# RobotLocomotion/pytorch-dense-correspondence

Measured on NVIDIA H100. Metric: image-pairs/s (640x480, D=3) fwd+loss+bwd, higher is better.
Workload: dtype f32 (bf16x3 split on the wgmma tensor cores, fp32 accumulate)

## Files before the change

pytorch-dense-correspondence_b200/csrc/conv_tc.cu:

```cuda
#include <cuda.h>
#include <algorithm>
#include <cstdlib>
#include <cstring>
#include <functional>
#include <mutex>
#include <unordered_map>

#include "conv.cuh"
#include "conv_tc.cuh"

namespace ddn {

constexpr int TC_BLOCK_K = 64;
constexpr int TC_CONSUMERS = 256;
constexpr int TC_THREADS = TC_CONSUMERS + 32;
constexpr int TC_PRODUCER_WARP = TC_CONSUMERS / 32;
constexpr int TC_WIDE_THREADS = TC_CONSUMERS + 128;
constexpr int TC_A_BYTES = 128 * TC_BLOCK_K * 2;

__device__ __forceinline__ uint32_t smem_u32(const void* p) { return (uint32_t)__cvta_generic_to_shared(p); }

__device__ __forceinline__ void mbar_init(uint32_t bar, uint32_t count) {
  asm volatile("mbarrier.init.shared::cta.b64 [%0], %1;" ::"r"(bar), "r"(count));
}
// ... 115 lines not shown
  } else {
    Wgmma<N>::template mma<TRANS>(d, a_hi, b_hi, accumulate);
  }
}
template <int N, int TRANS, int NPROD>
__device__ __forceinline__ void mma_k16_x(float (&d)[N / 2], float (&x)[N / 2], uint64_t a_hi, uint64_t a_lo, uint64_t b_hi, uint64_t b_lo,
                                          int accumulate) {
  if (NPROD == 3) {
    Wgmma<N>::template mma<TRANS>(x, a_hi, b_lo, accumulate);
    Wgmma<N>::template mma<TRANS>(x, a_lo, b_hi, 1);
  }
  Wgmma<N>::template mma<TRANS>(d, a_hi, b_hi, accumulate);
}
template <int K>
__device__ __forceinline__ void add_cross(float (&d)[K], const float (&x)[K]) {
#pragma unroll
  for (int i = 0; i < K; ++i) d[i] += x[i];
}
template <int N, int K>
__device__ __forceinline__ float (&acc_cols(float (&d)[K]))[N / 2] {
  static_assert(N / 2 <= K, "accumulator too narrow");
  return *reinterpret_cast<float(*)[N / 2]>(&d[0]);
}

constexpr int EPI_ROWS = 4;
constexpr int EPI_STRIDE = 40;
constexpr int EPI_WARP_FLOATS = 16 * EPI_STRIDE;

template <int K>
__device__ __forceinline__ void stage_write(const float (&acc)[K], int c, float* st, int lane) {
  const int r = lane >> 2, q = (lane & 3) * 2;
#pragma unroll
  for (int jj = 0; jj < 4; ++jj) {
    const int j = 4 * c + jj;
    *reinterpret_cast<float2*>(st + r * EPI_STRIDE + 8 * jj + q) = make_float2(acc[4 * j], acc[4 * j + 1]);
    *reinterpret_cast<float2*>(st + (r + 8) * EPI_STRIDE + 8 * jj + q) = make_float2(acc[4 * j + 2], acc[4 * j + 3]);
  }
  __syncwarp();
}

template <int K>
__device__ __forceinline__ void stage_chunk(const float (&acc)[K], int c, float* st, int lane, float4 (&v)[EPI_ROWS]) {
  stage_write(acc, c, st, lane);
  const int ga = lane >> 3, gb = lane & 7;
#pragma unroll
  for (int i = 0; i < EPI_ROWS; ++i) v[i] = *reinterpret_cast<const float4*>(st + (EPI_ROWS * ga + i) * EPI_STRIDE + 4 * gb);
  __syncwarp();
}

__device__ __forceinline__ uint32_t pack_bf16x2(__nv_bfloat16 a, __nv_bfloat16 b) {
  return (uint32_t)__bfloat16_as_ushort(a) | ((uint32_t)__bfloat16_as_ushort(b) << 16);
}

template <typename P>
__device__ __forceinline__ void conv_epilogue_rows(const P& p, const float4 (&v)[EPI_ROWS], size_t off, size_t rs, int n_ok, int ch,
                                                   int C, int grp, float4& s1, float4& s2) {
  float4 adv[EPI_ROWS];
#pragma unroll
  for (int i = 0; i < EPI_ROWS; ++i)
    adv[i] = (p.addend && i < n_ok) ? __ldg(reinterpret_cast<const float4*>(p.addend + off + i * rs)) : make_float4(0.f, 0.f, 0.f, 0.f);
  if (p.ep_scale) {
    const float4 sc = __ldg(reinterpret_cast<const float4*>(p.ep_scale + ch));
    const float4 sh = __ldg(reinterpret_cast<const float4*>(p.ep_shift + ch));
#pragma unroll
    for (int i = 0; i < EPI_ROWS; ++i) {
      float4 f = make_float4(fmaf(v[i].x, sc.x, sh.x) + adv[i].x, fmaf(v[i].y, sc.y, sh.y) + adv[i].y,
                             fmaf(v[i].z, sc.z, sh.z) + adv[i].z, fmaf(v[i].w, sc.w, sh.w) + adv[i].w);
      if (p.ep_relu) { f.x = fmaxf(f.x, 0.f); f.y = fmaxf(f.y, 0.f); f.z = fmaxf(f.z, 0.f); f.w = fmaxf(f.w, 0.f); }
      if (i < n_ok) {
        if (p.out) *reinterpret_cast<float4*>(p.out + off + i * rs) = f;
        if (p.out_hi) {
          const __nv_bfloat16 h0 = __float2bfloat16_rn(f.x), h1 = __float2bfloat16_rn(f.y), h2 = __float2bfloat16_rn(f.z), h3 = __float2bfloat16_rn(f.w);
          *reinterpret_cast<uint2*>(p.out_hi + off + i * rs) = make_uint2(pack_bf16x2(h0, h1), pack_bf16x2(h2, h3));
          if (p.out_lo)
            *reinterpret_cast<uint2*>(p.out_lo + off + i * rs) =
                make_uint2(pack_bf16x2(__float2bfloat16_rn(f.x - __bfloat162float(h0)), __float2bfloat16_rn(f.y - __bfloat162float(h1))),
                           pack_bf16x2(__float2bfloat16_rn(f.z - __bfloat162float(h2)), __float2bfloat16_rn(f.w - __bfloat162float(h3))));
        }
      }
    }
  } else if (p.bst.fin.a.acc) {
    float4 rw[EPI_ROWS];
    uint2 yh[EPI_ROWS];
#pragma unroll
    for (int i = 0; i < EPI_ROWS; ++i) {
      rw[i] = i < n_ok ? __ldg(reinterpret_cast<const float4*>(p.bst.raw + off + i * rs)) : make_float4(0.f, 0.f, 0.f, 0.f);
      if (p.bst.y_hi) yh[i] = i < n_ok ? __ldg(reinterpret_cast<const uint2*>(p.bst.y_hi + off + i * rs)) : make_uint2(0u, 0u);
    }
    const float4 mu = __ldg(reinterpret_cast<const float4*>(p.bst.mean + (size_t)grp * C + ch));
    const float4 is = __ldg(reinterpret_cast<const float4*>(p.bst.invstd + (size_t)grp * C + ch));
    float4 scl = make_float4(0.f, 0.f, 0.f, 0.f), be = scl;
    if (!p.bst.y_hi && p.bst.relu) {
      const float4 gm = __ldg(reinterpret_cast<const float4*>(p.bst.gamma + ch));
      be = __ldg(reinterpret_cast<const float4*>(p.bst.beta + ch));
      scl = make_float4(gm.x * is.x, gm.y * is.y, gm.z * is.z, gm.w * is.w);
    }
#pragma unroll
    for (int i = 0; i < EPI_ROWS; ++i) {
      float4 g = make_float4(v[i].x + adv[i].x, v[i].y + adv[i].y, v[i].z + adv[i].z, v[i].w + adv[i].w);
      if (i < n_ok) *reinterpret_cast<float4*>(p.out + off + i * rs) = g;
      else g = make_float4(0.f, 0.f, 0.f, 0.f);
      if (p.bst.y_hi) {
        const uint2 hh = yh[i];
        if ((hh.x & 0x8000u) || !(hh.x & 0x7fffu)) g.x = 0.f;
        if ((hh.x & 0x80000000u) || !(hh.x & 0x7fff0000u)) g.y = 0.f;
        if ((hh.y & 0x8000u) || !(hh.y & 0x7fffu)) g.z = 0.f;
        if ((hh.y & 0x80000000u) || !(hh.y & 0x7fff0000u)) g.w = 0.f;
      } else if (p.bst.relu) {
        if (!(fmaf(rw[i].x - mu.x, scl.x, be.x) > 0.f)) g.x = 0.f;
        if (!(fmaf(rw[i].y - mu.y, scl.y, be.y) > 0.f)) g.y = 0.f;
        if (!(fmaf(rw[i].z - mu.z, scl.z, be.z) > 0.f)) g.z = 0.f;
        if (!(fmaf(rw[i].w - mu.w, scl.w, be.w) > 0.f)) g.w = 0.f;
      }
      s1.x += g.x; s1.y += g.y; s1.z += g.z; s1.w += g.w;
      s2.x = fmaf(g.x, (rw[i].x - mu.x) * is.x, s2.x); s2.y = fmaf(g.y, (rw[i].y - mu.y) * is.y, s2.y);
      s2.z = fmaf(g.z, (rw[i].z - mu.z) * is.z, s2.z); s2.w = fmaf(g.w, (rw[i].w - mu.w) * is.w, s2.w);
    }
  } else {
#pragma unroll
    for (int i = 0; i < EPI_ROWS; ++i) {
      const float4 raw = i < n_ok ? v[i] : make_float4(0.f, 0.f, 0.f, 0.f);
      if (i < n_ok)
        *reinterpret_cast<float4*>(p.out + off + i * rs) = make_float4(raw.x + adv[i].x, raw.y + adv[i].y, raw.z + adv[i].z, raw.w + adv[i].w);
      s1.x += raw.x; s1.y += raw.y; s1.z += raw.z; s1.w += raw.w;
      s2.x = fmaf(raw.x, raw.x, s2.x); s2.y = fmaf(raw.y, raw.y, s2.y); s2.z = fmaf(raw.z, raw.z, s2.z); s2.w = fmaf(raw.w, raw.w, s2.w);
    }
  }
}

__device__ __forceinline__ void colsum_lane_groups(float4& s1, float4& s2) {
#pragma unroll
  for (int off = 8; off < 32; off <<= 1) {
    s1.x += __shfl_xor_sync(0xffffffffu, s1.x, off); s1.y += __shfl_xor_sync(0xffffffffu, s1.y, off);
    s1.z += __shfl_xor_sync(0xffffffffu, s1.z, off); s1.w += __shfl_xor_sync(0xffffffffu, s1.w, off);
    s2.x += __shfl_xor_sync(0xffffffffu, s2.x, off); s2.y += __shfl_xor_sync(0xffffffffu, s2.y, off);
    s2.z += __shfl_xor_sync(0xffffffffu, s2.z, off); s2.w += __shfl_xor_sync(0xffffffffu, s2.w, off);
  }
}

__device__ __forceinline__ void named_barrier(int id, int threads) { asm volatile("bar.sync %0, %1;" ::"r"(id), "r"(threads) : "memory"); }

struct TcConvParams {
  float* out;
  const float* addend;
  int N, H, W, Cin, Cout;
  int taps_w;
  int dil;
  int stride;
  int tiles_h, tiles_w;
  int n_sub;
  int n_co;
  int full_items, tail_split, total_items;
  int imgs_per_group;
  BnFwdFinal fin;
  TcBwdStats bst;
  const float* ep_scale; const float* ep_shift; int ep_relu;
  __nv_bfloat16* out_hi; __nv_bfloat16* out_lo;
};

constexpr int TC_SUB_H = 4, TC_SUB_W = 16;
constexpr int TC_SUB_BYTES = 64 * 128;

struct TcItem { int sp, co0, width; };
__device__ __forceinline__ TcItem tc_item(const TcConvParams& p, int idx, int block_n) {
  int tile = idx, piece = 0, width = block_n;
  if (idx >= p.full_items) {
    const int j = idx - p.full_items;
    tile = p.full_items + j / p.tail_split;
    piece = j - (j / p.tail_split) * p.tail_split;
    width = block_n / p.tail_split;
  }
  TcItem it;
  it.sp = tile / p.n_co;
  it.co0 = (tile - it.sp * p.n_co) * block_n + piece * width;
  it.width = width;
  return it;
}
struct TcSub { int n, h0, w0; bool valid; };
__device__ __forceinline__ TcSub tc_sub(const TcConvParams& p, int st) {
  TcSub s;
  s.valid = st < p.n_sub;
  const int tw = st % p.tiles_w; const int t = st / p.tiles_w;
  const int th = t % p.tiles_h;
  s.n = s.valid ? t / p.tiles_h : p.N;
  s.h0 = th * TC_SUB_H; s.w0 = tw * TC_SUB_W;
  return s;
}

template <int W, int BLOCK_N, int NPROD, int STAGES, int TRANS = 0>
__device__ __forceinline__ void conv_tc_mainloop(float (&acc)[W / 2], float (&accx)[W / 2], int num_kb, uint32_t& g, const uint64_t* full_bar,
                                                 const uint64_t* empty_bar, const uint8_t* smem, int wg, int lane) {
  constexpr int NSPLIT = NPROD == 3 ? 2 : 1;
  constexpr int A_BYTES = 128 * TC_BLOCK_K * 2;
  constexpr int B_BYTES = BLOCK_N * TC_BLOCK_K * 2;
  constexpr int STAGE_BYTES = NSPLIT * (A_BYTES + B_BYTES);
  constexpr uint32_t LBO = TRANS ? TC_SUB_BYTES : 16;
  constexpr int K_STEP = TRANS ? 16 * 128 : 32;
  for (int kb = 0; kb < num_kb; ++kb, ++g) {
    const int s = g % STAGES;
    mbar_wait(smem_u32(&full_bar[s]), (g / STAGES) & 1);
    wgmma_fence();
    const uint32_t stg = smem_u32(smem + (size_t)s * STAGE_BYTES);
    const uint64_t a_hi = gmma_desc(stg + wg * TC_SUB_BYTES, LBO, 1024), a_lo = gmma_desc(stg + A_BYTES + wg * TC_SUB_BYTES, LBO, 1024);
    const uint64_t b_hi = gmma_desc(stg + NSPLIT * A_BYTES, LBO, 1024), b_lo = gmma_desc(stg + 2 * A_BYTES + B_BYTES, LBO, 1024);
#pragma unroll
    for (int k = 0; k < TC_BLOCK_K / 16; ++k) {
      const uint64_t adv = (uint64_t)((k * K_STEP) >> 4);
      mma_k16_x<W, TRANS, NPROD>(acc, accx, a_hi + adv, a_lo + adv, b_hi + adv, b_lo + adv, (kb | k) != 0);
    }
    wgmma_commit();
    wgmma_wait<1>();
    if (kb > 0 && lane == 0) mbar_arrive(smem_u32(&empty_bar[(g - 1) % STAGES]));
  }
  wgmma_wait<0>();
  fence_acc(acc);
  if (NPROD == 3) { fence_acc(accx); add_cross(acc, accx); }
  if (lane == 0) mbar_arrive(smem_u32(&empty_bar[(g - 1) % STAGES]));
}

template <int BLOCK_N, int NPROD>
__global__ void __launch_bounds__(TC_WIDE_THREADS, 1)
conv_tc_kernel(const __grid_constant__ CUtensorMap tm_a_hi, const __grid_constant__ CUtensorMap tm_a_lo,
               const __grid_constant__ CUtensorMap tm_b_hi, const __grid_constant__ CUtensorMap tm_b_lo,
               const __grid_constant__ CUtensorMap tm_bt_hi, const __grid_constant__ CUtensorMap tm_bt_lo,
               const TcConvParams p) {
  constexpr int NSPLIT = NPROD == 3 ? 2 : 1;
  constexpr int A_BYTES = 128 * TC_BLOCK_K * 2;
  constexpr int B_BYTES = BLOCK_N * TC_BLOCK_K * 2;
  constexpr int STAGE_BYTES = NSPLIT * (A_BYTES + B_BYTES);
  constexpr int STAGES = (192 * 1024) / STAGE_BYTES >= 8 ? 8 : (192 * 1024) / STAGE_BYTES;
  static_assert(STAGES >= 2, "pipeline needs at least two stages");

  extern __shared__ __align__(1024) uint8_t smem_raw[];
  uint8_t* smem = reinterpret_cast<uint8_t*>((reinterpret_cast<uintptr_t>(smem_raw) + 1023) & ~uintptr_t(1023));
  __shared__ __align__(8) uint64_t full_bar[STAGES];
  __shared__ __align__(8) uint64_t empty_bar[STAGES];
  __shared__ int s_last;
  __shared__ __align__(16) float s_stage[TC_CONSUMERS / 32][EPI_WARP_FLOATS];
  __shared__ __align__(16) float s_part[2][2][4][BLOCK_N];

  pdl_trigger();
  const int warp = __shfl_sync(0xffffffffu, threadIdx.x >> 5, 0), lane = threadIdx.x & 31;
  const int cin_chunks = p.Cin / TC_BLOCK_K;
  const int num_kb = p.taps_w * p.taps_w * cin_chunks;
  const int half = p.taps_w >> 1;

  if (threadIdx.x == 0) {
    for (int s = 0; s < STAGES; ++s) { mbar_init(smem_u32(&full_bar[s]), 1); mbar_init(smem_u32(&empty_bar[s]), TC_CONSUMERS / 32); }
    fence_barrier_init();
    tma_prefetch_desc(&tm_a_hi); tma_prefetch_desc(&tm_b_hi); tma_prefetch_desc(&tm_bt_hi);
    if (NSPLIT == 2) { tma_prefetch_desc(&tm_a_lo); tma_prefetch_desc(&tm_b_lo); tma_prefetch_desc(&tm_bt_lo); }
  }
  __syncthreads();
  pdl_wait();

  if (warp >= TC_PRODUCER_WARP) {
    setmaxnreg_dec<40>();
    if (warp == TC_PRODUCER_WARP && lane == 0) {
      uint32_t g = 0;
      for (int idx = blockIdx.x; idx < p.total_items; idx += gridDim.x) {
        const TcItem it = tc_item(p, idx, BLOCK_N);
        const bool tail = it.width != BLOCK_N;
        const uint32_t stage_tx = (uint32_t)(NSPLIT * (A_BYTES + it.width * TC_BLOCK_K * 2));
        const CUtensorMap* mb_hi = tail ? &tm_bt_hi : &tm_b_hi;
        const CUtensorMap* mb_lo = tail ? &tm_bt_lo : &tm_b_lo;
        const TcSub s0 = tc_sub(p, it.sp * 2), s1 = tc_sub(p, it.sp * 2 + 1);
        for (int kb = 0; kb < num_kb; ++kb, ++g) {
          const int s = g % STAGES;
          mbar_wait(smem_u32(&empty_bar[s]), ((g / STAGES) & 1) ^ 1);
          const int tap = kb / cin_chunks, cc = kb - tap * cin_chunks;
          const int r = tap / p.taps_w, sx = tap - r * p.taps_w;
          const int dh = (r - half) * p.dil, dw = (sx - half) * p.dil;
          uint8_t* stg = smem + (size_t)s * STAGE_BYTES;
          const uint32_t bar = smem_u32(&full_bar[s]);
          mbar_expect_tx(bar, stage_tx);
          tma_load_4d(smem_u32(stg), &tm_a_hi, bar, cc * TC_BLOCK_K, s0.w0 * p.stride + dw, s0.h0 * p.stride + dh, s0.n);
          tma_load_4d(smem_u32(stg + TC_SUB_BYTES), &tm_a_hi, bar, cc * TC_BLOCK_K, s1.w0 * p.stride + dw, s1.h0 * p.stride + dh, s1.n);
          tma_load_2d(smem_u32(stg + NSPLIT * A_BYTES), mb_hi, bar, kb * TC_BLOCK_K, it.co0);
          if (NSPLIT == 2) {
            tma_load_4d(smem_u32(stg + A_BYTES), &tm_a_lo, bar, cc * TC_BLOCK_K, s0.w0 * p.stride + dw, s0.h0 * p.stride + dh, s0.n);
            tma_load_4d(smem_u32(stg + A_BYTES + TC_SUB_BYTES), &tm_a_lo, bar, cc * TC_BLOCK_K, s1.w0 * p.stride + dw, s1.h0 * p.stride + dh, s1.n);
            tma_load_2d(smem_u32(stg + 2 * A_BYTES + B_BYTES), mb_lo, bar, kb * TC_BLOCK_K, it.co0);
          }
        }
      }
    }
  } else {
    setmaxnreg_inc<232>();
    const int wg = warp >> 2, w = warp & 3, e = threadIdx.x & 127;
    const int ga = lane >> 3, gb = lane & 7;
    const bool stats = p.fin.a.acc != nullptr;
    const bool bstats = p.bst.fin.a.acc != nullptr;
    double* const sum_acc = bstats ? p.bst.fin.a.acc : p.fin.a.acc;
    float* const st = s_stage[warp];
    float acc[BLOCK_N / 2], accx[BLOCK_N / 2];
    uint32_t g = 0;
    for (int idx = blockIdx.x; idx < p.total_items; idx += gridDim.x) {
      const TcItem it = tc_item(p, idx, BLOCK_N);
      if (it.width == BLOCK_N)
        conv_tc_mainloop<BLOCK_N, BLOCK_N, NPROD, STAGES>(acc, accx, num_kb, g, full_bar, empty_bar, smem, wg, lane);
      else if (BLOCK_N > 64 && it.width == 64)
        conv_tc_mainloop<64, BLOCK_N, NPROD, STAGES>(acc_cols<64>(acc), acc_cols<64>(accx), num_kb, g, full_bar, empty_bar, smem, wg, lane);
      else
        conv_tc_mainloop<32, BLOCK_N, NPROD, STAGES>(acc_cols<32>(acc), acc_cols<32>(accx), num_kb, g, full_bar, empty_bar, smem, wg, lane);

      const TcSub sb = tc_sub(p, it.sp * 2 + wg);
      const int h = sb.h0 + w, w4 = sb.w0 + EPI_ROWS * ga;
      const int n_ok = (sb.valid && h < p.H) ? min(EPI_ROWS, p.W - w4) : 0;
      const size_t pix = ((size_t)(n_ok > 0 ? sb.n : 0) * p.H + (n_ok > 0 ? h : 0)) * p.W + (n_ok > 0 ? w4 : 0);
      const size_t cbase = pix * p.Cout + it.co0 + gb * 4;
      const int grp = sb.valid ? sb.n / p.imgs_per_group : 0;
#pragma unroll
      for (int c = 0; c < BLOCK_N / 32; ++c) {
        if (c < (it.width >> 5)) {
          float4 v[EPI_ROWS];
          stage_chunk(acc, c, st, lane, v);
          float4 s1 = make_float4(0.f, 0.f, 0.f, 0.f), s2 = s1;
          conv_epilogue_rows(p, v, cbase + c * 32, (size_t)p.Cout, n_ok, it.co0 + c * 32 + gb * 4, p.Cout, grp, s1, s2);
          if (stats || bstats) {
            colsum_lane_groups(s1, s2);
            if (ga == 0) {
              *reinterpret_cast<float4*>(&s_part[wg][0][w][c * 32 + gb * 4]) = s1;
              *reinterpret_cast<float4*>(&s_part[wg][1][w][c * 32 + gb * 4]) = s2;
            }
          }
        }
      }
      if (stats || bstats) {
        named_barrier(1 + wg, 128);
        if (sb.valid)
          for (int col = e; col < it.width; col += 128) {
#pragma unroll
            for (int k = 0; k < 2; ++k) {
              const float sum = s_part[wg][k][0][col] + s_part[wg][k][1][col] + s_part[wg][k][2][col] + s_part[wg][k][3][col];
              red_add_f64(sum_acc + (size_t)(grp * 2 + k) * p.Cout + it.co0 + col, (double)sum);
            }
          }
        named_barrier(1 + wg, 128);
      }
    }
    if (stats) {
      const bool last = bn_last_cta(p.fin.a.ticket, gridDim.x, threadIdx.x == 0, &s_last, [] { named_barrier(3, TC_CONSUMERS); });
      if (last)
        for (int c = threadIdx.x; c < p.Cout; c += TC_CONSUMERS) bn_fwd_finalize_channel(p.fin, c);
    } else if (bstats) {
      const bool last = bn_last_cta(p.bst.fin.a.ticket, gridDim.x, threadIdx.x == 0, &s_last, [] { named_barrier(3, TC_CONSUMERS); });
      if (last)
        for (int c = threadIdx.x; c < p.Cout; c += TC_CONSUMERS) bn_bwd_finalize_channel(p.bst.fin, c);
    }
  }
}

struct TcHaloParams {
  float* out; const float* addend;
  int N, H, W;
  int tiles_h, tiles_w, n_tiles;
  int imgs_per_group;
  BnFwdFinal fin;
  TcBwdStats bst;
  const float* ep_scale; const float* ep_shift; int ep_relu;
  __nv_bfloat16* out_hi; __nv_bfloat16* out_lo;
};
constexpr int HALO_TH = 8, HALO_TW = 16;
constexpr int HALO_BH = HALO_TH + 2, HALO_BW = HALO_TW + 2;
constexpr int HALO_BOX_BYTES = HALO_BH * HALO_BW * 128;
constexpr int HALO_SLOT = ((HALO_BOX_BYTES + 1023) / 1024) * 1024;
constexpr int HALO_B_TAP = 64 * 128;
constexpr int HALO_B_PLANE = 9 * HALO_B_TAP;
__host__ __device__ constexpr int halo_slots(int nprod) { return nprod == 3 ? 2 : 3; }

template <int NPROD>
__global__ void __launch_bounds__(TC_THREADS, 1)
conv64_halo_kernel(const __grid_constant__ CUtensorMap tm_a_hi, const __grid_constant__ CUtensorMap tm_a_lo,
                   const __grid_constant__ CUtensorMap tm_b_hi, const __grid_constant__ CUtensorMap tm_b_lo, const TcHaloParams p) {
  constexpr int NSPLIT = NPROD == 3 ? 2 : 1;
  constexpr int SLOTS = halo_slots(NPROD);
  extern __shared__ __align__(1024) uint8_t smem_raw[];
  uint8_t* smem = reinterpret_cast<uint8_t*>((reinterpret_cast<uintptr_t>(smem_raw) + 1023) & ~uintptr_t(1023));
  uint8_t* smem_b = smem;
  uint8_t* smem_a = smem + NSPLIT * HALO_B_PLANE;
  __shared__ __align__(8) uint64_t full_bar[SLOTS], empty_bar[SLOTS], b_full;
  __shared__ int s_last;
  __shared__ __align__(16) float s_stage[TC_CONSUMERS / 32][EPI_WARP_FLOATS];
  __shared__ __align__(16) float s_part[2][8][64];

  pdl_trigger();
  const int warp = __shfl_sync(0xffffffffu, threadIdx.x >> 5, 0), lane = threadIdx.x & 31;
  if (threadIdx.x == 0) {
    for (int s = 0; s < SLOTS; ++s) { mbar_init(smem_u32(&full_bar[s]), 1); mbar_init(smem_u32(&empty_bar[s]), TC_CONSUMERS / 32); }
    mbar_init(smem_u32(&b_full), 1);
    fence_barrier_init();
    tma_prefetch_desc(&tm_a_hi); tma_prefetch_desc(&tm_b_hi);
    if (NSPLIT == 2) { tma_prefetch_desc(&tm_a_lo); tma_prefetch_desc(&tm_b_lo); }
  }
  __syncthreads();
  pdl_wait();

  auto tile_of = [&](int t, int& n, int& h0, int& w0) {
    const int tw = t % p.tiles_w; const int q = t / p.tiles_w;
    const int th = q % p.tiles_h; n = q / p.tiles_h;
    h0 = th * HALO_TH; w0 = tw * HALO_TW;
  };

  if (warp == TC_PRODUCER_WARP) {
    if (lane == 0) {
      const uint32_t bb = smem_u32(&b_full);
      mbar_expect_tx(bb, NSPLIT * HALO_B_PLANE);
#pragma unroll 1
      for (int tap = 0; tap < 9; ++tap) {
        tma_load_2d(smem_u32(smem_b + tap * HALO_B_TAP), &tm_b_hi, bb, tap * 64, 0);
        if (NSPLIT == 2) tma_load_2d(smem_u32(smem_b + HALO_B_PLANE + tap * HALO_B_TAP), &tm_b_lo, bb, tap * 64, 0);
      }
      uint32_t g = 0;
      constexpr int PF = 2;
      for (int j = 0; j < PF; ++j) {
        const int tp = blockIdx.x + j * gridDim.x;
        if (tp < p.n_tiles) {
          int n, h0, w0;
          tile_of(tp, n, h0, w0);
          tma_prefetch_l2_4d(&tm_a_hi, 0, h0 - 1, w0 - 1, n);
          if (NSPLIT == 2) tma_prefetch_l2_4d(&tm_a_lo, 0, h0 - 1, w0 - 1, n);
        }
      }
      for (int t = blockIdx.x; t < p.n_tiles; t += gridDim.x) {
        int n, h0, w0;
        {
          const int tp = t + PF * gridDim.x;
          if (tp < p.n_tiles) {
            tile_of(tp, n, h0, w0);
            tma_prefetch_l2_4d(&tm_a_hi, 0, h0 - 1, w0 - 1, n);
            if (NSPLIT == 2) tma_prefetch_l2_4d(&tm_a_lo, 0, h0 - 1, w0 - 1, n);
          }
        }
        tile_of(t, n, h0, w0);
#pragma unroll
        for (int pl = 0; pl < NSPLIT; ++pl, ++g) {
          const int s = g % SLOTS;
          mbar_wait(smem_u32(&empty_bar[s]), ((g / SLOTS) & 1) ^ 1);
          const uint32_t bar = smem_u32(&full_bar[s]);
          mbar_expect_tx(bar, HALO_BOX_BYTES);
          tma_load_4d(smem_u32(smem_a + s * HALO_SLOT), pl == 0 ? &tm_a_hi : &tm_a_lo, bar, 0, h0 - 1, w0 - 1, n);
        }
      }
    }
  } else {
    const int wg = warp >> 2, w = warp & 3;
    const int ga = lane >> 3, gb = lane & 7;
    const bool stats = p.fin.a.acc != nullptr;
    const bool bstats = p.bst.fin.a.acc != nullptr;
    double* const sum_acc = bstats ? p.bst.fin.a.acc : p.fin.a.acc;
    float* const st = s_stage[warp];
    mbar_wait(smem_u32(&b_full), 0);
    const uint64_t bd_hi = gmma_desc_k(smem_u32(smem_b));
    const uint64_t bd_lo = gmma_desc_k(smem_u32(smem_b + HALO_B_PLANE));
    const uint32_t a_wg = (uint32_t)(8 * wg * HALO_BH * 128);
    float acc[32], accx[32];
    uint32_t g = 0;
    for (int t = blockIdx.x; t < p.n_tiles; t += gridDim.x) {
      int n, h0, w0;
      tile_of(t, n, h0, w0);
      const int s_hi = g % SLOTS;
      {
        mbar_wait(smem_u32(&full_bar[s_hi]), (g / SLOTS) & 1);
        wgmma_fence();
        const uint64_t a0 = gmma_desc_k(smem_u32(smem_a + s_hi * HALO_SLOT) + a_wg, HALO_BH * 128);
#pragma unroll
        for (int tap = 0; tap < 9; ++tap) {
#pragma unroll
          for (int k = 0; k < 4; ++k) {
            const uint64_t ad = a0 + (uint64_t)((((tap % 3) * HALO_BH + tap / 3) * 128 + k * 32) >> 4);
            const uint64_t boff = (uint64_t)((tap * HALO_B_TAP + k * 32) >> 4);
            if (NPROD == 3) Wgmma<64>::mma<0>(accx, ad, bd_lo + boff, (tap | k) != 0);
            Wgmma<64>::mma<0>(acc, ad, bd_hi + boff, (tap | k) != 0);
          }
        }
        wgmma_commit();
        ++g;
      }
      if (NPROD == 3) {
        const int s = g % SLOTS;
        mbar_wait(smem_u32(&full_bar[s]), (g / SLOTS) & 1);
        const uint64_t a0 = gmma_desc_k(smem_u32(smem_a + s * HALO_SLOT) + a_wg, HALO_BH * 128);
#pragma unroll
        for (int tap = 0; tap < 9; ++tap) {
#pragma unroll
          for (int k = 0; k < 4; ++k)
            Wgmma<64>::mma<0>(accx, a0 + (uint64_t)((((tap % 3) * HALO_BH + tap / 3) * 128 + k * 32) >> 4),
                              bd_hi + (uint64_t)((tap * HALO_B_TAP + k * 32) >> 4), 1);
        }
        wgmma_commit();
        wgmma_wait<1>();
        if (lane == 0) mbar_arrive(smem_u32(&empty_bar[s_hi]));
        ++g;
      }
      wgmma_wait<0>();
      fence_acc(acc);
      if (NPROD == 3) { fence_acc(accx); add_cross(acc, accx); }
      if (lane == 0) mbar_arrive(smem_u32(&empty_bar[(g - 1) % SLOTS]));

      const size_t pix0 = ((size_t)n * p.H + h0 + EPI_ROWS * (ga & 1)) * p.W + (w0 + 8 * wg + 2 * w + (ga >> 1));
      const size_t row_stride = (size_t)p.W * 64;
      const int grp = n / p.imgs_per_group;
#pragma unroll
      for (int c = 0; c < 2; ++c) {
        float4 v[EPI_ROWS];
        stage_chunk(acc, c, st, lane, v);
        float4 s1 = make_float4(0.f, 0.f, 0.f, 0.f), s2 = s1;
        conv_epilogue_rows(p, v, pix0 * 64 + gb * 4 + c * 32, row_stride, EPI_ROWS, c * 32 + gb * 4, 64, grp, s1, s2);
        if (stats || bstats) {
          colsum_lane_groups(s1, s2);
          if (ga == 0) {
            *reinterpret_cast<float4*>(&s_part[0][warp][c * 32 + gb * 4]) = s1;
            *reinterpret_cast<float4*>(&s_part[1][warp][c * 32 + gb * 4]) = s2;
          }
        }
      }
      if (stats || bstats) {
        named_barrier(3, TC_CONSUMERS);
        if (threadIdx.x < 128) {
          const int col = threadIdx.x & 63, k = threadIdx.x >> 6;
          float s8 = 0.f;
#pragma unroll
          for (int q = 0; q < 8; ++q) s8 += s_part[k][q][col];
          red_add_f64(sum_acc + (size_t)(grp * 2 + k) * 64 + col, (double)s8);
        }
        named_barrier(3, TC_CONSUMERS);
      }
    }
    if (bstats) {
      const bool last = bn_last_cta(p.bst.fin.a.ticket, gridDim.x, threadIdx.x == 0, &s_last, [] { named_barrier(3, TC_CONSUMERS); });
      if (last)
        for (int c = threadIdx.x; c < 64; c += TC_CONSUMERS) bn_bwd_finalize_channel(p.bst.fin, c);
    } else if (stats) {
      const bool last = bn_last_cta(p.fin.a.ticket, gridDim.x, threadIdx.x == 0, &s_last, [] { named_barrier(3, TC_CONSUMERS); });
      if (last)
        for (int c = threadIdx.x; c < 64; c += TC_CONSUMERS) bn_fwd_finalize_channel(p.fin, c);
    }
  }
}

struct TcWgradParams {
  double* dwp;
  int N, H, W, Cin, Cout;
  int taps_w, dil, stride;
  int tiles_h, tiles_w;
  int total_kb;
  int n_co, n_ci, n_tiles;
  int chunks;
};

struct WgradItem { int co0, ci0, tap, kb0, kb1; };
__device__ __forceinline__ WgradItem wgrad_item(const TcWgradParams& p, int idx, int bn) {
  const int c = idx / p.n_tiles;
  int t = idx - c * p.n_tiles;
  WgradItem it;
  it.co0 = (t % p.n_co) * 128; t /= p.n_co;
  it.ci0 = (t % p.n_ci) * bn;
  it.tap = t / p.n_ci;
  it.kb0 = (int)((int64_t)c * p.total_kb / p.chunks);
  it.kb1 = (int)((int64_t)(c + 1) * p.total_kb / p.chunks);
  return it;
// ... 641 lines not shown
  return fold != 0;
}

bool tc_conv_supported(int Cin, int Cout, int k, int stride, int pad, int dil, int H, int W) {
  if (Cin % 64 || Cout % 64) return false;
  if (stride == 2) { if (dil != 1 || (H & 1) || (W & 1)) return false; }
  else if (stride != 1) return false;
  if (k == 3) return pad == dil;
  if (k == 1) return pad == 0;
  return false;
}

static const size_t kMaxWeightElems = (size_t)9 * 512 * 512;
size_t tc_weight_ws_bytes() { return 2 * align_up(kMaxWeightElems * 2, 1024) + 2048; }

int tc_split(const float* x, __nv_bfloat16* hi, __nv_bfloat16* lo, int64_t n, int precision, cudaStream_t st) {
  DDN_CHECK_ARG(n % 4 == 0, "split: element count must be a multiple of 4");
  int64_t n4 = n / 4;
  int blocks = (int)std::min<int64_t>(ceil_div(n4, 256), (int64_t)num_sms() * 8);
  DDN_LAUNCH(split_bf16_kernel, blocks, 256, 0, st, x, hi, lo, n4, precision == DDN_PRECISION_BF16X3 ? 1 : 0);
  return 0;
}

int tc_pack_weights(const float* w_oihw, __nv_bfloat16* hi, __nv_bfloat16* lo, int Cout, int Cin, int k, int dgrad, int precision,
                    cudaStream_t st) {
  const size_t wel = (size_t)Cout * Cin * k * k;
  int wblocks = (int)std::min<int64_t>(ceil_div((int64_t)wel, 256), 4096);
  DDN_LAUNCH(pack_weights_tc_kernel, wblocks, 256, 0, st, w_oihw, hi, lo, Cout, Cin, k, dgrad, precision == DDN_PRECISION_BF16X3 ? 1 : 0);
  return 0;
}

int tc_upsample_zero_split(const float* dy, __nv_bfloat16* hi, __nv_bfloat16* lo, int N, int Ho, int Wo, int C, int precision,
                           cudaStream_t st) {
  int64_t total = (int64_t)N * Ho * Wo * (C / 4);
  int blocks = (int)std::min<int64_t>(ceil_div(total, 256), (int64_t)num_sms() * 8);
  DDN_LAUNCH(upsample_zero_split_kernel, blocks, 256, 0, st, dy, hi, lo, N, Ho, Wo, C, precision == DDN_PRECISION_BF16X3 ? 1 : 0);
  return 0;
}

int tc_stem_patches(const float* x_nchw, __nv_bfloat16* hi, __nv_bfloat16* lo, int N, int H, int W, int precision, cudaStream_t st) {
  const int H1 = (H - 1) / 2 + 1, W1 = (W - 1) / 2 + 1;
  DDN_CHECK_ARG(N <= 65535 && H1 <= 65535, "stem: batch / height too large for the launch grid");
  dim3 grid((unsigned)ceil_div(W1, STEM_TW), (unsigned)H1, (unsigned)N);
  DDN_LAUNCH(stem_patch_split_kernel, grid, 256, 0, st, x_nchw, hi, lo, N, H, W, H1, W1, precision == DDN_PRECISION_BF16X3 ? 1 : 0);
  return 0;
}

static bool tc_tail_enabled() {
  static int v = -1;
  if (v < 0) { const char* e = getenv("DDN_TC_TAIL"); v = (e && e[0] == '0') ? 0 : 1; }
  return v != 0;
}

template <int BLOCK_N, int NPROD>
static int launch_conv_tc(const CUtensorMap& a_hi, const CUtensorMap& a_lo, const CUtensorMap& b_hi, const CUtensorMap& b_lo,
                          const CUtensorMap& bt_hi, const CUtensorMap& bt_lo, const TcConvParams& p, int workers, cudaStream_t st) {
  constexpr int NSPLIT = NPROD == 3 ? 2 : 1;
  constexpr int STAGE_BYTES = NSPLIT * (128 * TC_BLOCK_K * 2 + BLOCK_N * TC_BLOCK_K * 2);
  constexpr int STAGES = (192 * 1024) / STAGE_BYTES >= 8 ? 8 : (192 * 1024) / STAGE_BYTES;
  const size_t smem = (size_t)STAGES * STAGE_BYTES + 1024;
  static bool configured = false;
  if (!configured) {
    DDN_CUDA(cudaFuncSetAttribute(conv_tc_kernel<BLOCK_N, NPROD>, cudaFuncAttributeMaxDynamicSharedMemorySize, (int)smem));
    configured = true;
  }
  DDN_LAUNCH((conv_tc_kernel<BLOCK_N, NPROD>), workers, TC_WIDE_THREADS, smem, st, a_hi, a_lo, b_hi, b_lo, bt_hi, bt_lo, p);
  return 0;
}

template <int NPROD>
static int launch_conv64_halo(const CUtensorMap& a_hi, const CUtensorMap& a_lo, const CUtensorMap& b_hi, const CUtensorMap& b_lo,
                              const TcHaloParams& p, cudaStream_t st) {
  constexpr int NSPLIT = NPROD == 3 ? 2 : 1;
  const size_t smem = (size_t)NSPLIT * HALO_B_PLANE + (size_t)halo_slots(NPROD) * HALO_SLOT + 1024;
  static bool configured = false;
  if (!configured) {
    DDN_CUDA(cudaFuncSetAttribute(conv64_halo_kernel<NPROD>, cudaFuncAttributeMaxDynamicSharedMemorySize, (int)smem));
    configured = true;
  }
  const int grid = std::min(p.n_tiles, tc_worker_sms());
  DDN_LAUNCH((conv64_halo_kernel<NPROD>), grid, TC_THREADS, smem, st, a_hi, a_lo, b_hi, b_lo, p);
  return 0;
}

int tc_conv_planes(TcPlanes in, const float* w_oihw, const TcPlanes* wpk, float* out, const float* addend, const BnFwdFinal* stats,
                   int N, int H, int W, int Cin, int Cout, int k, int stride, int dil, int dgrad, int precision,
                   void* wws, size_t wws_bytes, cudaStream_t st, const TcFoldedEpilogue* ep, const TcBwdStats* bst) {
  DDN_CHECK_ARG(stride == 1 || !dgrad, "the strided data gradient goes through zero-inserted planes (stride 1 here)");
  const int Ho = H / stride, Wo = W / stride;
  const double fl = 2.0 * N * Ho * Wo * (double)Cout * k * k * Cin;
  const int gin = dgrad ? Cout : Cin, gout = dgrad ? Cin : Cout;
  const int want_lo = precision == DDN_PRECISION_BF16X3;
  const __nv_bfloat16* b_hi; const __nv_bfloat16* b_lo;
  if (wpk) {
    b_hi = wpk->hi; b_lo = wpk->lo;
  } else {
    const size_t wel = (size_t)Cout * Cin * k * k;
    const size_t w_b = align_up(kMaxWeightElems * 2, 1024);
    DDN_CHECK_ARG(wws != nullptr && wel <= kMaxWeightElems, "tc weight staging missing or weight tensor too large");
    char* base = reinterpret_cast<char*>(align_up(reinterpret_cast<uintptr_t>(wws), 1024));
    if ((size_t)(base - (char*)wws) + 2 * w_b > wws_bytes) { set_error("tensor-core weight staging too small"); return DDN_EWORKSPACE; }
    __nv_bfloat16* ph = (__nv_bfloat16*)base; __nv_bfloat16* pl = (__nv_bfloat16*)(base + w_b);
    int wblocks = (int)std::min<int64_t>(ceil_div((int64_t)wel, 256), 4096);
    DDN_LAUNCH(pack_weights_tc_kernel, wblocks, 256, 0, st, w_oihw, ph, pl, Cout, Cin, k, dgrad, want_lo);
    b_hi = ph; b_lo = pl;
  }
  if (tc_halo_enabled() && k == 3 && gin == 64 && gout == 64 && stride == 1 && dil == 1 && Ho % HALO_TH == 0 && Wo % HALO_TW == 0) {
    TcHaloParams hp;
    memset(&hp, 0, sizeof(hp));
    if (ep) {
      DDN_CHECK_ARG(!dgrad && !stats && !bst && ep->scale && ep->shift && (out || ep->out_hi), "folded epilogue: forward only, needs scale/shift and an output");
      hp.ep_scale = ep->scale; hp.ep_shift = ep->shift; hp.ep_relu = ep->relu; hp.out_hi = ep->out_hi; hp.out_lo = want_lo ? ep->out_lo : nullptr;
    } else {
      DDN_CHECK_ARG(out != nullptr, "conv output pointer is null");
    }
    hp.out = out; hp.addend = addend; hp.N = N; hp.H = Ho; hp.W = Wo;
    hp.tiles_h = Ho / HALO_TH; hp.tiles_w = Wo / HALO_TW; hp.n_tiles = N * hp.tiles_h * hp.tiles_w;
    hp.imgs_per_group = N;
    if (stats) {
      DDN_CHECK_ARG(!dgrad && stats->G >= 1 && stats->G <= BN_MAX_GROUPS && N % stats->G == 0 && stats->C == 64, "bad BatchNorm statistics request");
      hp.fin = *stats;
      hp.imgs_per_group = N / stats->G;
    }
    if (bst) {
      DDN_CHECK_ARG(dgrad && !stats && bst->raw && bst->mean && bst->invstd && bst->fin.a.acc && bst->fin.G >= 1 && bst->fin.G <= BN_MAX_GROUPS &&
                    N % bst->fin.G == 0 && bst->fin.C == 64 && (bst->y_hi || !bst->relu || (bst->gamma && bst->beta)),
                    "bad BatchNorm backward-statistics request");
      hp.bst = *bst;
      hp.imgs_per_group = N / bst->fin.G;
    }
    CUtensorMap ma_hi, ma_lo, mb_hi, mb_lo;
    DDN_TRY(make_act_map_halo(&ma_hi, in.hi, N, H, W, 64));
    DDN_TRY(make_act_map_halo(&ma_lo, want_lo ? in.lo : in.hi, N, H, W, 64));
    DDN_TRY(make_weight_map(&mb_hi, b_hi, 64, 9 * 64, 64));
    DDN_TRY(make_weight_map(&mb_lo, want_lo ? b_lo : b_hi, 64, 9 * 64, 64));
    ProfScope ps(dgrad ? PROF_CONV_DGRAD_TC : PROF_CONV_FWD_TC, fl, st);
    return want_lo ? launch_conv64_halo<3>(ma_hi, ma_lo, mb_hi, mb_lo, hp, st) : launch_conv64_halo<1>(ma_hi, ma_lo, mb_hi, mb_lo, hp, st);
  }
  const int block_n = gout % 128 == 0 ? 128 : 64;
  TcConvParams p;
  memset(&p, 0, sizeof(p));
  p.out = out; p.addend = addend; p.N = N; p.H = Ho; p.W = Wo; p.Cin = gin; p.Cout = gout; p.taps_w = k; p.dil = dil;
  p.stride = stride;
  p.tiles_h = (int)ceil_div(Ho, TC_SUB_H); p.tiles_w = (int)ceil_div(Wo, TC_SUB_W);
  p.n_sub = N * p.tiles_h * p.tiles_w;
  p.n_co = gout / block_n;
  const int tiles = (int)ceil_div(p.n_sub, 2) * p.n_co;
  const int workers_max = tc_worker_sms();
  const int rem = tiles % workers_max;
  int split = 1;
  if (rem && tc_tail_enabled())
    while (split * 2 <= 8 && block_n / (split * 2) >= 32 && rem * split * 2 <= workers_max) split *= 2;
  p.full_items = tiles - rem; p.tail_split = split; p.total_items = p.full_items + rem * split;
  if (split == 1) { p.full_items = tiles; p.total_items = tiles; }
  const int workers = std::min(p.total_items, workers_max);
  p.imgs_per_group = N;
  if (stats) {
    DDN_CHECK_ARG(!dgrad && !ep && stats->G >= 1 && stats->G <= BN_MAX_GROUPS && N % stats->G == 0, "bad BatchNorm statistics request");
    p.fin = *stats;
    p.imgs_per_group = N / stats->G;
  }
  if (bst) {
    DDN_CHECK_ARG(dgrad && !ep && !stats && bst->raw && bst->mean && bst->invstd && bst->fin.a.acc && bst->fin.G >= 1 &&
                  bst->fin.G <= BN_MAX_GROUPS && N % bst->fin.G == 0 && bst->fin.C == gout && (bst->y_hi || !bst->relu || (bst->gamma && bst->beta)),
                  "bad BatchNorm backward-statistics request");
    p.bst = *bst;
    p.imgs_per_group = N / bst->fin.G;
  }
  if (ep) {
    DDN_CHECK_ARG(!dgrad && !stats && ep->scale && ep->shift && (out || ep->out_hi), "folded epilogue: forward only, needs scale/shift and an output");
    p.ep_scale = ep->scale; p.ep_shift = ep->shift; p.ep_relu = ep->relu; p.out_hi = ep->out_hi; p.out_lo = want_lo ? ep->out_lo : nullptr;
  } else {
    DDN_CHECK_ARG(out != nullptr, "conv output pointer is null");
  }
  const int b_rows = block_n;
  const int bt_rows = b_rows / split;
  CUtensorMap ma_hi, ma_lo, mb_hi, mb_lo, mt_hi, mt_lo;
  DDN_TRY(make_act_map(&ma_hi, in.hi, N, H, W, gin, stride));
  DDN_TRY(make_act_map(&ma_lo, want_lo ? in.lo : in.hi, N, H, W, gin, stride));
  DDN_TRY(make_weight_map(&mb_hi, b_hi, gout, k * k * gin, b_rows));
  DDN_TRY(make_weight_map(&mb_lo, want_lo ? b_lo : b_hi, gout, k * k * gin, b_rows));
  DDN_TRY(make_weight_map(&mt_hi, b_hi, gout, k * k * gin, bt_rows));
  DDN_TRY(make_weight_map(&mt_lo, want_lo ? b_lo : b_hi, gout, k * k * gin, bt_rows));
  ProfScope ps(dgrad ? PROF_CONV_DGRAD_TC : PROF_CONV_FWD_TC, fl, st);
#define CONV_TC(BN)                                                                                                           \
  (want_lo ? launch_conv_tc<BN, 3>(ma_hi, ma_lo, mb_hi, mb_lo, mt_hi, mt_lo, p, workers, st)                                   \
           : launch_conv_tc<BN, 1>(ma_hi, ma_lo, mb_hi, mb_lo, mt_hi, mt_lo, p, workers, st))
  if (block_n == 128) return CONV_TC(128);
  return CONV_TC(64);
#undef CONV_TC
}

int tc_dgrad_strided(const float* dy_f32, TcPlanes up, const float* w_oihw, const TcPlanes* w_packed, float* dx, const float* addend,
                     int N, int H, int W, int Cin, int Cout, int k, int precision, void* wws, size_t wws_bytes, cudaStream_t st,
                     const TcBwdStats* bst) {
  DDN_TRY(tc_upsample_zero_split(dy_f32, const_cast<__nv_bfloat16*>(up.hi), const_cast<__nv_bfloat16*>(up.lo), N, H / 2, W / 2, Cout,
                                 precision, st));
  return tc_conv_planes(up, w_oihw, w_packed, dx, addend, nullptr, N, H, W, Cin, Cout, k, 1, 1, 1, precision, wws, wws_bytes, st, nullptr, bst);
}

int tc_stem_pack_weights(const float* w_conv1, __nv_bfloat16* hi, __nv_bfloat16* lo, int precision, cudaStream_t st) {
  DDN_LAUNCH(stem_pack_weights_kernel, (64 * 192 + 255) / 256, 256, 0, st, w_conv1, hi, lo, precision == DDN_PRECISION_BF16X3 ? 1 : 0);
  return 0;
}
int tc_stem_forward(TcPlanes patches, const float* w_conv1, const TcPlanes* w_packed, float* raw, const BnFwdFinal* stats, int N, int H1,
                    int W1, int precision, void* wws, size_t wws_bytes, cudaStream_t st) {
  TcPlanes wpk;
  if (w_packed) wpk = *w_packed;
  else {
    char* base = reinterpret_cast<char*>(align_up(reinterpret_cast<uintptr_t>(wws), 1024));
    DDN_CHECK_ARG((size_t)(base - (char*)wws) + 2 * 64 * 192 * 2 + 1024 <= wws_bytes, "weight staging too small");
    __nv_bfloat16* ph = (__nv_bfloat16*)base; __nv_bfloat16* pl = (__nv_bfloat16*)(base + align_up((size_t)64 * 192 * 2, 1024));
    DDN_TRY(tc_stem_pack_weights(w_conv1, ph, pl, precision, st));
    wpk.hi = ph; wpk.lo = pl;
  }
  return tc_conv_planes(patches, nullptr, &wpk, raw, nullptr, stats, N, H1, W1, 192, 64, 1, 1, 1, 0, precision, wws, wws_bytes, st);
}

int tc_stem_wgrad(TcPlanes patches, TcPlanes dy, float* dw_conv1, int N, int H1, int W1, int precision, double* scratch, cudaStream_t st) {
  if (!dw_conv1) return tc_wgrad_planes(patches, dy, nullptr, N, H1, W1, 192, 64, 1, 1, 1, precision, scratch, st);
  double* dwp = scratch; float* dwk = reinterpret_cast<float*>(scratch + 64 * 192);
  DDN_TRY(tc_wgrad_planes(patches, dy, dwk, N, H1, W1, 192, 64, 1, 1, 1, precision, dwp, st));
  DDN_LAUNCH(stem_unpack_wgrad_kernel, (64 * 147 + 255) / 256, 256, 0, st, dwk, dw_conv1);
  return 0;
}

int tc_pack_all(const float* params, int64_t n_params, char* cache, const TcPackEntry* entries, int n, unsigned long long* fp_new,
                unsigned long long* fp_old, int force, int precision, cudaStream_t st) {
  DDN_CHECK_ARG(n >= 1 && n <= TC_PACK_MAX, "pack table too large");
  TcPackTable t; t.n = n;
  for (int i = 0; i < n; ++i) t.e[i] = entries[i];
  DDN_LAUNCH(param_fingerprint_kernel, num_sms() * 2, 256, 0, st, reinterpret_cast<const uint32_t*>(params), n_params, fp_new);
  dim3 grid(32, (unsigned)n);
  DDN_LAUNCH(pack_all_kernel, grid, 256, 0, st, params, cache, t, fp_new, fp_old, force, precision == DDN_PRECISION_BF16X3 ? 1 : 0);
  DDN_LAUNCH(commit_fingerprint_kernel, 1, 32, 0, st, fp_new, fp_old);
  return 0;
}

size_t tc_workspace_bytes(size_t max_act_elems) { return tc_weight_ws_bytes() + 6 * align_up(max_act_elems * 2, 1024) + 4096; }

// ... 45 lines not shown
```

Baseline: 139.6.

## Prefetch dgrad epilogue operands before the mainloop and one chunk ahead

Splits the epilogue's global loads (addend, raw activations, bf16 y_hi mask) into a separate epi_load step. For dgrad launches (PIPE=true), the loads for the first chunk are issued before the wgmma mainloop and the next chunk's loads during the current chunk's epilogue. This hides global-memory latency behind tensor-core work. Keeping the prefetched values live across the mainloop adds register pressure, which is why the 128-wide bf16x3 variant is excluded.

```diff
diff --git a/pytorch-dense-correspondence_b200/csrc/conv_tc.cu b/pytorch-dense-correspondence_b200/csrc/conv_tc.cu
--- a/pytorch-dense-correspondence_b200/csrc/conv_tc.cu
+++ b/pytorch-dense-correspondence_b200/csrc/conv_tc.cu
@@ -191,13 +191,29 @@
   return (uint32_t)__bfloat16_as_ushort(a) | ((uint32_t)__bfloat16_as_ushort(b) << 16);
 }
 
+struct EpiIn { float4 adv[EPI_ROWS]; float4 rw[EPI_ROWS]; uint2 yh[EPI_ROWS]; };
+
 template <typename P>
-__device__ __forceinline__ void conv_epilogue_rows(const P& p, const float4 (&v)[EPI_ROWS], size_t off, size_t rs, int n_ok, int ch,
-                                                   int C, int grp, float4& s1, float4& s2) {
-  float4 adv[EPI_ROWS];
-#pragma unroll
-  for (int i = 0; i < EPI_ROWS; ++i)
-    adv[i] = (p.addend && i < n_ok) ? __ldg(reinterpret_cast<const float4*>(p.addend + off + i * rs)) : make_float4(0.f, 0.f, 0.f, 0.f);
+__device__ __forceinline__ void epi_load(const P& p, size_t off, size_t rs, int n_ok, EpiIn& in) {
+#pragma unroll
+  for (int i = 0; i < EPI_ROWS; ++i) {
+    in.adv[i] = (p.addend && i < n_ok) ? __ldg(reinterpret_cast<const float4*>(p.addend + off + i * rs)) : make_float4(0.f, 0.f, 0.f, 0.f);
+    in.rw[i] = make_float4(0.f, 0.f, 0.f, 0.f);
+    in.yh[i] = make_uint2(0u, 0u);
+  }
+  if (!p.ep_scale && p.bst.fin.a.acc) {
+#pragma unroll
+    for (int i = 0; i < EPI_ROWS; ++i) {
+      if (i < n_ok) in.rw[i] = __ldg(reinterpret_cast<const float4*>(p.bst.raw + off + i * rs));
+      if (p.bst.y_hi && i < n_ok) in.yh[i] = __ldg(reinterpret_cast<const uint2*>(p.bst.y_hi + off + i * rs));
+    }
+  }
+}
+
+template <typename P>
+__device__ __forceinline__ void conv_epilogue_rows(const P& p, const float4 (&v)[EPI_ROWS], const EpiIn& in, size_t off, size_t rs, int n_ok,
+                                                   int ch, int C, int grp, float4& s1, float4& s2) {
+  const float4 (&adv)[EPI_ROWS] = in.adv;
   if (p.ep_scale) {
     const float4 sc = __ldg(reinterpret_cast<const float4*>(p.ep_scale + ch));
     const float4 sh = __ldg(reinterpret_cast<const float4*>(p.ep_shift + ch));
@@ -219,13 +235,8 @@
       }
     }
   } else if (p.bst.fin.a.acc) {
-    float4 rw[EPI_ROWS];
-    uint2 yh[EPI_ROWS];
-#pragma unroll
-    for (int i = 0; i < EPI_ROWS; ++i) {
-      rw[i] = i < n_ok ? __ldg(reinterpret_cast<const float4*>(p.bst.raw + off + i * rs)) : make_float4(0.f, 0.f, 0.f, 0.f);
-      if (p.bst.y_hi) yh[i] = i < n_ok ? __ldg(reinterpret_cast<const uint2*>(p.bst.y_hi + off + i * rs)) : make_uint2(0u, 0u);
-    }
+    const float4 (&rw)[EPI_ROWS] = in.rw;
+    const uint2 (&yh)[EPI_ROWS] = in.yh;
     const float4 mu = __ldg(reinterpret_cast<const float4*>(p.bst.mean + (size_t)grp * C + ch));
     const float4 is = __ldg(reinterpret_cast<const float4*>(p.bst.invstd + (size_t)grp * C + ch));
     float4 scl = make_float4(0.f, 0.f, 0.f, 0.f), be = scl;
@@ -316,6 +327,7 @@
   return it;
 }
 struct TcSub { int n, h0, w0; bool valid; };
+struct TcEpiPos { size_t cbase; int n_ok, grp; bool valid; };
 __device__ __forceinline__ TcSub tc_sub(const TcConvParams& p, int st) {
   TcSub s;
   s.valid = st < p.n_sub;
@@ -357,7 +369,7 @@
   if (lane == 0) mbar_arrive(smem_u32(&empty_bar[(g - 1) % STAGES]));
 }
 
-template <int BLOCK_N, int NPROD>
+template <int BLOCK_N, int NPROD, bool PIPE>
 __global__ void __launch_bounds__(TC_WIDE_THREADS, 1)
 conv_tc_kernel(const __grid_constant__ CUtensorMap tm_a_hi, const __grid_constant__ CUtensorMap tm_a_lo,
                const __grid_constant__ CUtensorMap tm_b_hi, const __grid_constant__ CUtensorMap tm_b_lo,
@@ -436,26 +448,42 @@
     uint32_t g = 0;
     for (int idx = blockIdx.x; idx < p.total_items; idx += gridDim.x) {
       const TcItem it = tc_item(p, idx, BLOCK_N);
+      const auto locate = [&](TcEpiPos& e) {
+        const TcSub sb = tc_sub(p, it.sp * 2 + wg);
+        const int h = sb.h0 + w, w4 = sb.w0 + EPI_ROWS * ga;
+        e.valid = sb.valid;
+        e.n_ok = (sb.valid && h < p.H) ? min(EPI_ROWS, p.W - w4) : 0;
+        const size_t pix = ((size_t)(e.n_ok > 0 ? sb.n : 0) * p.H + (e.n_ok > 0 ? h : 0)) * p.W + (e.n_ok > 0 ? w4 : 0);
+        e.cbase = pix * p.Cout + it.co0 + gb * 4;
+        e.grp = sb.valid ? sb.n / p.imgs_per_group : 0;
+      };
+      constexpr bool kEarly = PIPE && !(BLOCK_N == 128 && NPROD == 3);
+      const int nch = it.width >> 5;
+      TcEpiPos ep;
+      EpiIn in;
+      if (kEarly) { locate(ep); epi_load(p, ep.cbase, (size_t)p.Cout, ep.n_ok, in); }
       if (it.width == BLOCK_N)
         conv_tc_mainloop<BLOCK_N, BLOCK_N, NPROD, STAGES>(acc, accx, num_kb, g, full_bar, empty_bar, smem, wg, lane);
       else if (BLOCK_N > 64 && it.width == 64)
         conv_tc_mainloop<64, BLOCK_N, NPROD, STAGES>(acc_cols<64>(acc), acc_cols<64>(accx), num_kb, g, full_bar, empty_bar, smem, wg, lane);
       else
         conv_tc_mainloop<32, BLOCK_N, NPROD, STAGES>(acc_cols<32>(acc), acc_cols<32>(accx), num_kb, g, full_bar, empty_bar, smem, wg, lane);
-
-      const TcSub sb = tc_sub(p, it.sp * 2 + wg);
-      const int h = sb.h0 + w, w4 = sb.w0 + EPI_ROWS * ga;
-      const int n_ok = (sb.valid && h < p.H) ? min(EPI_ROWS, p.W - w4) : 0;
-      const size_t pix = ((size_t)(n_ok > 0 ? sb.n : 0) * p.H + (n_ok > 0 ? h : 0)) * p.W + (n_ok > 0 ? w4 : 0);
-      const size_t cbase = pix * p.Cout + it.co0 + gb * 4;
-      const int grp = sb.valid ? sb.n / p.imgs_per_group : 0;
+      if (!kEarly) locate(ep);
+      const size_t cbase = ep.cbase;
+      const int n_ok = ep.n_ok, grp = ep.grp;
+
 #pragma unroll
       for (int c = 0; c < BLOCK_N / 32; ++c) {
-        if (c < (it.width >> 5)) {
+        if (c < nch) {
+          const bool ahead = kEarly && c + 1 < BLOCK_N / 32 && c + 1 < nch;
+          if (!kEarly) epi_load(p, cbase + c * 32, (size_t)p.Cout, n_ok, in);
           float4 v[EPI_ROWS];
           stage_chunk(acc, c, st, lane, v);
+          EpiIn next;
+          if (ahead) epi_load(p, cbase + (c + 1) * 32, (size_t)p.Cout, n_ok, next);
           float4 s1 = make_float4(0.f, 0.f, 0.f, 0.f), s2 = s1;
-          conv_epilogue_rows(p, v, cbase + c * 32, (size_t)p.Cout, n_ok, it.co0 + c * 32 + gb * 4, p.Cout, grp, s1, s2);
+          conv_epilogue_rows(p, v, in, cbase + c * 32, (size_t)p.Cout, n_ok, it.co0 + c * 32 + gb * 4, p.Cout, grp, s1, s2);
+          if (ahead) in = next;
           if (stats || bstats) {
             colsum_lane_groups(s1, s2);
             if (ga == 0) {
@@ -467,7 +495,7 @@
       }
       if (stats || bstats) {
         named_barrier(1 + wg, 128);
-        if (sb.valid)
+        if (ep.valid)
           for (int col = e; col < it.width; col += 128) {
 #pragma unroll
             for (int k = 0; k < 2; ++k) {
@@ -508,7 +536,7 @@
 constexpr int HALO_B_PLANE = 9 * HALO_B_TAP;
 __host__ __device__ constexpr int halo_slots(int nprod) { return nprod == 3 ? 2 : 3; }
 
-template <int NPROD>
+template <int NPROD, bool PIPE>
 __global__ void __launch_bounds__(TC_THREADS, 1)
 conv64_halo_kernel(const __grid_constant__ CUtensorMap tm_a_hi, const __grid_constant__ CUtensorMap tm_a_lo,
                    const __grid_constant__ CUtensorMap tm_b_hi, const __grid_constant__ CUtensorMap tm_b_lo, const TcHaloParams p) {
@@ -598,6 +626,11 @@
     for (int t = blockIdx.x; t < p.n_tiles; t += gridDim.x) {
       int n, h0, w0;
       tile_of(t, n, h0, w0);
+      const size_t pix0 = ((size_t)n * p.H + h0 + EPI_ROWS * (ga & 1)) * p.W + (w0 + 8 * wg + 2 * w + (ga >> 1));
+      const size_t row_stride = (size_t)p.W * 64;
+      const int grp = n / p.imgs_per_group;
+      EpiIn in;
+      if (PIPE) epi_load(p, pix0 * 64 + gb * 4, row_stride, EPI_ROWS, in);
       const int s_hi = g % SLOTS;
       {
         mbar_wait(smem_u32(&full_bar[s_hi]), (g / SLOTS) & 1);
@@ -637,15 +670,16 @@
       if (NPROD == 3) { fence_acc(accx); add_cross(acc, accx); }
       if (lane == 0) mbar_arrive(smem_u32(&empty_bar[(g - 1) % SLOTS]));
 
-      const size_t pix0 = ((size_t)n * p.H + h0 + EPI_ROWS * (ga & 1)) * p.W + (w0 + 8 * wg + 2 * w + (ga >> 1));
-      const size_t row_stride = (size_t)p.W * 64;
-      const int grp = n / p.imgs_per_group;
 #pragma unroll
       for (int c = 0; c < 2; ++c) {
+        if (!PIPE) epi_load(p, pix0 * 64 + gb * 4 + c * 32, row_stride, EPI_ROWS, in);
         float4 v[EPI_ROWS];
         stage_chunk(acc, c, st, lane, v);
+        EpiIn next;
+        if (PIPE && c == 0) epi_load(p, pix0 * 64 + gb * 4 + 32, row_stride, EPI_ROWS, next);
         float4 s1 = make_float4(0.f, 0.f, 0.f, 0.f), s2 = s1;
-        conv_epilogue_rows(p, v, pix0 * 64 + gb * 4 + c * 32, row_stride, EPI_ROWS, c * 32 + gb * 4, 64, grp, s1, s2);
+        conv_epilogue_rows(p, v, in, pix0 * 64 + gb * 4 + c * 32, row_stride, EPI_ROWS, c * 32 + gb * 4, 64, grp, s1, s2);
+        if (PIPE && c == 0) in = next;
         if (stats || bstats) {
           colsum_lane_groups(s1, s2);
           if (ga == 0) {
@@ -1393,7 +1427,7 @@
   return v != 0;
 }
 
-template <int BLOCK_N, int NPROD>
+template <int BLOCK_N, int NPROD, bool PIPE>
 static int launch_conv_tc(const CUtensorMap& a_hi, const CUtensorMap& a_lo, const CUtensorMap& b_hi, const CUtensorMap& b_lo,
                           const CUtensorMap& bt_hi, const CUtensorMap& bt_lo, const TcConvParams& p, int workers, cudaStream_t st) {
   constexpr int NSPLIT = NPROD == 3 ? 2 : 1;
@@ -1402,25 +1436,25 @@
   const size_t smem = (size_t)STAGES * STAGE_BYTES + 1024;
   static bool configured = false;
   if (!configured) {
-    DDN_CUDA(cudaFuncSetAttribute(conv_tc_kernel<BLOCK_N, NPROD>, cudaFuncAttributeMaxDynamicSharedMemorySize, (int)smem));
+    DDN_CUDA(cudaFuncSetAttribute(conv_tc_kernel<BLOCK_N, NPROD, PIPE>, cudaFuncAttributeMaxDynamicSharedMemorySize, (int)smem));
     configured = true;
   }
-  DDN_LAUNCH((conv_tc_kernel<BLOCK_N, NPROD>), workers, TC_WIDE_THREADS, smem, st, a_hi, a_lo, b_hi, b_lo, bt_hi, bt_lo, p);
+  DDN_LAUNCH((conv_tc_kernel<BLOCK_N, NPROD, PIPE>), workers, TC_WIDE_THREADS, smem, st, a_hi, a_lo, b_hi, b_lo, bt_hi, bt_lo, p);
   return 0;
 }
 
-template <int NPROD>
+template <int NPROD, bool PIPE>
 static int launch_conv64_halo(const CUtensorMap& a_hi, const CUtensorMap& a_lo, const CUtensorMap& b_hi, const CUtensorMap& b_lo,
                               const TcHaloParams& p, cudaStream_t st) {
   constexpr int NSPLIT = NPROD == 3 ? 2 : 1;
   const size_t smem = (size_t)NSPLIT * HALO_B_PLANE + (size_t)halo_slots(NPROD) * HALO_SLOT + 1024;
   static bool configured = false;
   if (!configured) {
-    DDN_CUDA(cudaFuncSetAttribute(conv64_halo_kernel<NPROD>, cudaFuncAttributeMaxDynamicSharedMemorySize, (int)smem));
+    DDN_CUDA(cudaFuncSetAttribute(conv64_halo_kernel<NPROD, PIPE>, cudaFuncAttributeMaxDynamicSharedMemorySize, (int)smem));
     configured = true;
   }
   const int grid = std::min(p.n_tiles, tc_worker_sms());
-  DDN_LAUNCH((conv64_halo_kernel<NPROD>), grid, TC_THREADS, smem, st, a_hi, a_lo, b_hi, b_lo, p);
+  DDN_LAUNCH((conv64_halo_kernel<NPROD, PIPE>), grid, TC_THREADS, smem, st, a_hi, a_lo, b_hi, b_lo, p);
   return 0;
 }
 
@@ -1476,7 +1510,9 @@
     DDN_TRY(make_weight_map(&mb_hi, b_hi, 64, 9 * 64, 64));
     DDN_TRY(make_weight_map(&mb_lo, want_lo ? b_lo : b_hi, 64, 9 * 64, 64));
     ProfScope ps(dgrad ? PROF_CONV_DGRAD_TC : PROF_CONV_FWD_TC, fl, st);
-    return want_lo ? launch_conv64_halo<3>(ma_hi, ma_lo, mb_hi, mb_lo, hp, st) : launch_conv64_halo<1>(ma_hi, ma_lo, mb_hi, mb_lo, hp, st);
+    if (dgrad)
+      return want_lo ? launch_conv64_halo<3, true>(ma_hi, ma_lo, mb_hi, mb_lo, hp, st) : launch_conv64_halo<1, true>(ma_hi, ma_lo, mb_hi, mb_lo, hp, st);
+    return want_lo ? launch_conv64_halo<3, false>(ma_hi, ma_lo, mb_hi, mb_lo, hp, st) : launch_conv64_halo<1, false>(ma_hi, ma_lo, mb_hi, mb_lo, hp, st);
   }
   const int block_n = gout % 128 == 0 ? 128 : 64;
   TcConvParams p;
@@ -1525,8 +1561,10 @@
   DDN_TRY(make_weight_map(&mt_lo, want_lo ? b_lo : b_hi, gout, k * k * gin, bt_rows));
   ProfScope ps(dgrad ? PROF_CONV_DGRAD_TC : PROF_CONV_FWD_TC, fl, st);
 #define CONV_TC(BN)                                                                                                           \
-  (want_lo ? launch_conv_tc<BN, 3>(ma_hi, ma_lo, mb_hi, mb_lo, mt_hi, mt_lo, p, workers, st)                                   \
-           : launch_conv_tc<BN, 1>(ma_hi, ma_lo, mb_hi, mb_lo, mt_hi, mt_lo, p, workers, st))
+  (dgrad ? (want_lo ? launch_conv_tc<BN, 3, true>(ma_hi, ma_lo, mb_hi, mb_lo, mt_hi, mt_lo, p, workers, st)                    \
+                    : launch_conv_tc<BN, 1, true>(ma_hi, ma_lo, mb_hi, mb_lo, mt_hi, mt_lo, p, workers, st))                   \
+         : (want_lo ? launch_conv_tc<BN, 3, false>(ma_hi, ma_lo, mb_hi, mb_lo, mt_hi, mt_lo, p, workers, st)                   \
+                    : launch_conv_tc<BN, 1, false>(ma_hi, ma_lo, mb_hi, mb_lo, mt_hi, mt_lo, p, workers, st)))
   if (block_n == 128) return CONV_TC(128);
   return CONV_TC(64);
 #undef CONV_TC
```

Result: no change. 140.2, median of 6 (+0.4%).
